# MiRaCLeXeoN/sduss

Measured on AMD Instinct MI355X. Metric: images/sec (node), SDXL 1024^2 50-step, fixed prompt, CFG, higher is better.
Workload: dtype bf16; 1 GPU; SDXL-base-1.0 UNet 1024x1024 50-step Euler, CFG 5.0, 4 requests/step (denoiser batch 8) per GPU, is_sliced=False, random-init weights of the real architecture (2.57 B params), one data-parallel replica per GPU, no collective; resolution=1024, steps_per_image=50

## Files before the change

include/mxdenoise.h:

```cpp
#ifndef MXDENOISE_H
#define MXDENOISE_H

#include <stddef.h>
#include <stdint.h>

#ifdef __cplusplus
extern "C" {
#endif

enum { MX_F32 = 0, MX_F16 = 1, MX_BF16 = 2 };

const char* mx_last_error(void);
int mx_version(void);
#define MX_PROF_KINDS 12
int mx_profile_enable(int on);
int mx_profile_collect(double* out);
int mx_profile_records(double* out, int max_records);

size_t mx_groupnorm_halo_workspace_bytes(int N, int C, int cpg);
int mx_groupnorm_halo(void* stream, const void* x, const void* gamma, const void* beta, void* y,
                      int N, int C, int H, int W, int cpg, double eps, int padding,
                      const int32_t* latent_offset, int n_latents, const int32_t* patch_map,
                      const int32_t* padding_idx, int dtype, void* workspace);
int mx_halo_only(void* stream, const void* x, void* y, int N, int C, int H, int W,
// ... 43 lines not shown
  int lda, ldc, ldr, ldrb;
  int rows_per_batch;
  int flags;
  int seg, period, ldvt;
  int B, Hin, Win, Cin;
  int Hout, Wout;
  int stride;
  int up;
  int corner_patch;
  int a_batch_rows, a_row_off, c_batch_rows, c_row_off;
  const float* gate;
  int ldg;
  float out_scale;
  const float* rms_wq;
  const float* rms_wk;
  float rms_eps;
  int vhalo;
  const void* a2;
  int lda2, k_split;
  const float* ln_stats;
  const float* ln_colsum;
  int ln_slabs;
  float ln_eps;
  float* stats_out;
  const mx_gemm_seg* segs;
  int n_segs;
  int splitk;
  const float* ln_final;
  float* ln_final_out;
  unsigned* ln_final_cnt;
  float* gn_part_out;
  int cin_valid;
} mx_gemm_desc;

int mx_gemm(void* stream, const mx_gemm_desc* d);
int mx_gemm_launches(const mx_gemm_desc* d);
int mx_gemm_stats_slabs(const mx_gemm_desc* d);
int mx_gemm_ln_prefers_pass(const mx_gemm_desc* d);
int mx_gemm_ln_final_supported(const mx_gemm_desc* d);
int mx_gemm_gn_partials_supported(const mx_gemm_desc* d, int conv);
enum { MX_LN_ROUTES_PATCH_PARALLEL = 1, MX_LN_ROUTES_PATCH_CACHE = 2, MX_LN_ROUTES_TICKETS = 4 };
int mx_unet_ln_routes(int M, int C, int layers, int n_groups, int flags, int routes[4]);
enum { MX_FORM_TILE_GENERIC = 0, MX_FORM_TILE_256 = 1, MX_FORM_TILE_128 = 2, MX_FORM_PERSISTENT_256 = 3, MX_FORM_SMALL_M = 4, MX_FORM_CONV_SMALL_N = 5, MX_FORM_CONV_SMALL_CIN = 6 };
int mx_gemm_form(const mx_gemm_desc* d, int conv);
int mx_gemm_kernel_name(const mx_gemm_desc* d, int conv, int launch, char* buf, int cap);
int mx_gemm_kernel_names(char* buf, int cap);
int mx_attention_kernel_name(int B, int H, int Lq, int Lk, int ldo, int prescaled, int causal, int bias, int key_chunk, int force_cross, char* buf, int cap);
int mx_attention_kernel_names(char* buf, int cap);
#define MX_STATS_PITCH(slabs) (((slabs) + 3) & ~3)
int mx_row_stats(void* stream, const void* x, int ldx, float* stats, int M, int C);
int mx_conv3x3(void* stream, const mx_gemm_desc* d);
int mx_conv3x3_halo_serves(const mx_gemm_desc* d);
int mx_conv3x3_halo(void* stream, const mx_gemm_desc* d);
int mx_gemm_splitk(const mx_gemm_desc* d, int conv);
void mx_gemm_release_scratch(void* stream, int all);

#define MX_VT_POS(key) (((key) & ~12) | (((key) & 4) << 1) | (((key) & 8) >> 1))
#define MX_VT_LD(Lk) (((Lk) + 15) / 16 * 16)

int mx_attention(void* stream, const void* q, int ldq, const void* k, int ldk, const void* vt, int ldvt,
                 int64_t vt_batch_stride, void* o, int ldo, int B, int H, int Lq, int Lk, float scale);
#define MX_ATTN_QSCALE(scale) ((scale) * 1.4426950408889634f)
int mx_attention_prescaled(void* stream, const void* q, int ldq, const void* k, int ldk, const void* vt, int ldvt,
                           int64_t vt_batch_stride, void* o, int ldo, int B, int H, int Lq, int Lk);
int mx_attention_cross_prescaled(void* stream, const void* q, int ldq, const void* k, int ldk, const void* vt, int ldvt,
                                 int64_t vt_batch_stride, void* o, int ldo, int B, int H, int Lq, int Lk);
typedef struct mx_attn_problem {
  const void* q; const void* k; const void* vt; void* o;
  int64_t vt_batch_stride;
  int B, Lq, Lk, ldvt;
} mx_attn_problem;
int mx_attention_prescaled_grouped(void* stream, const mx_attn_problem* probs, int n, int ldq, int ldk, int ldo, int H);
int mx_attention_prescaled_bias(void* stream, const void* q, int ldq, const void* k, int ldk, const void* vt, int ldvt,
                                int64_t vt_batch_stride, void* o, int ldo, int B, int H, int Lq, int Lk, const float* bias, int ldb);
int mx_attention_prescaled_causal(void* stream, const void* q, int ldq, const void* k, int ldk, const void* vt, int ldvt,
                                  int64_t vt_batch_stride, void* o, int ldo, int B, int H, int L);

int mx_layernorm(void* stream, const void* x, void* y, const float* gamma, const float* beta,
                 int M, int C, float eps);

int mx_rmsnorm(void* stream, const void* x, void* y, const float* w, int M, int C, float eps);

int mx_layernorm_mod(void* stream, const void* x, void* y, void* y2, const float* scale, const float* shift,
                     const float* scale2, const float* shift2, int ldmod, int M, int C, int rows_per_batch, float eps);
int mx_layernorm_mod_grouped(void* stream, const void* x, void* y, void* y2, const float* scale, const float* shift, const float* scale2,
                             const float* shift2, int ldmod, int C, float eps, const int* batches, const int* rows_per_batch, int n);
int mx_rmsnorm_heads(void* stream, void* x, int ld, int nbatch, int rows_per_batch, int batch_rows, int row_off,
                     int heads_total, int heads_q, const float* wq, const float* wk, float eps, float q_scale);

size_t mx_groupnorm_nhwc_workspace_bytes(int B, int H, int W, int C);
int mx_groupnorm_nhwc(void* stream, const void* x, void* y, const float* gamma, const float* beta,
                      int B, int H, int W, int C, int groups, float eps, int silu, int patch,
                      void* workspace);

int mx_groupnorm_nhwc_cat(void* stream, const void* x, int C1, const void* x2, void* y, const float* gamma, const float* beta,
                          int B, int H, int W, int C, int groups, float eps, int silu, int patch, void* workspace);
int mx_groupnorm_nhwc_from_partials(void* stream, const void* x, void* y, const float* gamma, const float* beta, int B, int H, int W, int C, int groups, float eps,
                                    int silu, const float* part, int chunk, const float* add_bias, const float* add_rowbias, int ldrb, void* workspace);

typedef struct mx_gn_problem { const void* x; const void* x2; void* y; int B, H, W; } mx_gn_problem;
size_t mx_groupnorm_nhwc_grouped_workspace_bytes(const mx_gn_problem* probs, int n, int C);
int mx_groupnorm_nhwc_grouped(void* stream, const mx_gn_problem* probs, int n, int C1, const float* gamma, const float* beta, int C, int groups,
                              float eps, int silu, int patch, void* workspace);

typedef struct mx_unet_config {
  int in_channels, out_channels;
// ... 358 lines not shown
```

sduss_amd/csrc/conv_halo.hip:

```cpp
#include "common.h"
#include "../../include/mxdenoise.h"
#include "gemm_args.h"
#include "gemm_dma_loader.h"

#include <type_traits>

namespace mx {

constexpr int HALO_BN = 160;
constexpr int HALO_WSTAGE_BYTES = HALO_BN * DMA_BK * 2;
constexpr int HALO_ZERO_BYTES = 256;
__host__ __device__ constexpr int halo_lines(int W) { return (256 / W + 2) * W; }
__host__ __device__ constexpr int halo_xbuf_bytes(int W) { return halo_lines(W) * DMA_BK * 2; }
__host__ __device__ constexpr int halo_lds_bytes(int W) { return 2 * halo_xbuf_bytes(W) + 3 * HALO_WSTAGE_BYTES + HALO_ZERO_BYTES; }

template <int W, bool VEC>
__global__ __launch_bounds__(512, 2) void conv_halo_kernel(const GemmArgs pk) {
  constexpr int BN = HALO_BN, MI = 4, NI = BN / 32;
  constexpr int LINES = halo_lines(W);
  constexpr int XBUF = halo_xbuf_bytes(W);
  constexpr int XN = LINES * 8 / 512;
  constexpr int WCH = BN * 8, WI = 3;
  constexpr int WRING = 2 * XBUF, ZERO = WRING + 3 * HALO_WSTAGE_BYTES;
  static_assert(W == 32 || W == 64, "a tile is whole image rows of 32 or 64 pixels");
  static_assert(LINES * 8 % 512 == 0 && XBUF % 256 == 0, "whole DMA instructions; buffers keep the bank half of a line");
  __shared__ __attribute__((aligned(256))) char smem[halo_lds_bytes(W)];

  const GemmArgs& p = pk;
  int tm, tn;
  gemm_tile_of_block(blockIdx.x, p.M / 256, p.N / BN, p.xcd_map, tm, tn);
  const int tid = threadIdx.x;
  const int lane = tid & 63;
  const int wave = __builtin_amdgcn_readfirstlane(tid >> 6);
  const int wm = wave >> 1;
  const int wn = wave & 1;
  const bool group_b = wave >= 4;
  const int cs = tid & 7;
  const int nchunks = p.Cin / DMA_BK;
  const char* zero = reinterpret_cast<const char*>(g_zero_page);

  const int m0 = tm * 256, n0 = tn * BN;
  const int hw = p.Hin * p.Win;
  const int img = m0 / hw;
  const int y0 = (m0 - img * hw) / W;
  const char* xsrc[XN];
#pragma unroll
  for (int i = 0; i < XN; ++i) {
    const int P = (i * 512 + tid) >> 3;
    const int sr = P / W, x = P - sr * W;
    const int iy = y0 - 1 + sr;
    const bool ok = iy >= 0 && iy < p.Hin;
    const long off = (((long)img * p.Hin + iy) * W + x) * (long)p.Cin * 2;
    xsrc[i] = (ok ? reinterpret_cast<const char*>(p.a) + off : zero) + swz(P, cs) * 16;
  }
  const char* wsrc[WI];
#pragma unroll
  for (int i = 0; i < WI; ++i) {
    int q = i * 512 + tid;
    if (q >= WCH) q -= WCH;
    const int row = q >> 3;
    wsrc[i] = reinterpret_cast<const char*>(p.w) + ((long)(n0 + row) * p.K + swz(row, cs) * 8) * 2;
  }
  const long w_tap_step = (long)p.Cin * 2, w_chunk_step = DMA_BK * 2 - 8 * (long)p.Cin * 2;

  auto issue_x = [&](int buf, int i) __attribute__((always_inline)) {
    glds16(xsrc[i], smem + buf * XBUF + (i * 512 + wave * 64) * 16);
  };
  auto advance_x = [&](int next_chunk) __attribute__((always_inline)) {
#pragma unroll
    for (int i = 0; i < XN; ++i) xsrc[i] = next_chunk < nchunks ? xsrc[i] + DMA_BK * 2 : zero + lane * 16;
  };
  auto issue_w = [&](int stage) __attribute__((always_inline)) {
#pragma unroll
    for (int i = 0; i < WI; ++i) {
      const int qb = (i * 512 + wave * 64 >= WCH) ? i * 512 + wave * 64 - WCH : i * 512 + wave * 64;
      glds16(wsrc[i], smem + WRING + stage * HALO_WSTAGE_BYTES + qb * 16);
    }
  };
  auto step_w = [&](long step) __attribute__((always_inline)) {
#pragma unroll
    for (int i = 0; i < WI; ++i) wsrc[i] += step;
  };
  auto to_next_chunk_w = [&](bool last) __attribute__((always_inline)) {
#pragma unroll
    for (int i = 0; i < WI; ++i) wsrc[i] = last ? zero + lane * 16 : wsrc[i] + w_chunk_step;
  };

  const int fr = lane & 15;
  const int fq = lane >> 4;
  unsigned wrd[2];
  unsigned xrd[3][2];
  unsigned zrd[3][2];
#pragma unroll
  for (int ks = 0; ks < 2; ++ks) {
    const int wrow = wn * (BN / 2) + fr;
    wrd[ks] = (unsigned)(WRING + wrow * 128 + swz(wrow, ks * 4 + fq) * 16);
#pragma unroll
    for (int d = 0; d < 3; ++d) {
      const int line = wm * 64 + fr + d - 1;
      const int key = ((fr + d - 1) >> 1) & 7;
      const int rel = line * 128 + ((ks * 4 + fq) ^ key) * 16;
      xrd[d][ks] = (unsigned)rel;
      zrd[d][ks] = (unsigned)(ZERO + (rel & 255));
    }
  }
  const bool lane_left = fr == 0, lane_right = fr == 15;

  if (tid < HALO_ZERO_BYTES / 16) *reinterpret_cast<u32x4*>(smem + ZERO + tid * 16) = u32x4{0u, 0u, 0u, 0u};

#pragma unroll
  for (int i = 0; i < XN; ++i) issue_x(0, i);
  advance_x(1);
  issue_w(0); step_w(w_tap_step);
  issue_w(1); step_w(w_tap_step);
  wait_vmcnt<WI>();

  f32x4 acc[NI][MI];
#pragma unroll
  for (int i = 0; i < NI; ++i)
#pragma unroll
    for (int j = 0; j < MI; ++j) acc[i][j] = f32x4{0.f, 0.f, 0.f, 0.f};
  float ln_rstd[MI];
#pragma unroll
  for (int j = 0; j < MI; ++j) ln_rstd[j] = 1.0f;
  asm volatile("s_waitcnt lgkmcnt(0)" ::: "memory");
  MX_BAR();
  if (group_b) MX_BAR();

  for (int cc = 0; cc < nchunks; ++cc) {
    const int cur = cc & 1, nxt = cur ^ 1;
    const unsigned xb = (unsigned)(cur * XBUF);
    const bool last = cc + 1 == nchunks;
    auto phase = [&](auto tc) __attribute__((always_inline)) {
      constexpr int T = decltype(tc)::value;
      constexpr int dy = T / 3 - 1, dx = T % 3 - 1, d = dx + 1;
      bf16x8 wf[2][NI], xf[2][MI];
#pragma unroll
      for (int ks = 0; ks < 2; ++ks) {
#pragma unroll
        for (int i = 0; i < NI; ++i) wf[ks][i] = *reinterpret_cast<const bf16x8*>(smem + wrd[ks] + (T % 3) * HALO_WSTAGE_BYTES + i * (16 * 128));
#pragma unroll
        for (int j = 0; j < MI; ++j) {
          unsigned a = xb + xrd[d][ks] + (unsigned)((dy + 1) * W * 128 + j * (16 * 128));
          if (dx == -1 && (j * 16) % W == 0) a = lane_left ? zrd[d][ks] : a;
          if (dx == 1 && (j * 16 + 16) % W == 0) a = lane_right ? zrd[d][ks] : a;
          xf[ks][j] = *reinterpret_cast<const bf16x8*>(smem + a);
        }
      }
      int nx = 0;
#pragma unroll
      for (int i = 0; i < XN; ++i)
        if ((i * 7) / (XN - 1) == T) { issue_x(nxt, i); ++nx; }
      issue_w((T + 2) % 3);
      if (T == 6) to_next_chunk_w(last);
      else step_w(T > 6 && last ? 0 : w_tap_step);
      if (T == 8) advance_x(cc + 2);
      if (nx == 0) wait_vmcnt<WI>(); else if (nx == 1) wait_vmcnt<WI + 1>(); else wait_vmcnt<WI + 2>();
      asm volatile("s_waitcnt lgkmcnt(0)" ::: "memory");
      __builtin_amdgcn_sched_barrier(0);
      MX_BAR();
      __builtin_amdgcn_s_setprio(1);
#pragma unroll
      for (int ks = 0; ks < 2; ++ks)
#pragma unroll
        for (int i = 0; i < NI; ++i)
#pragma unroll
          for (int j = 0; j < MI; ++j) acc[i][j] = __builtin_amdgcn_mfma_f32_16x16x32_bf16(wf[ks][i], xf[ks][j], acc[i][j], 0, 0, 0);
      __builtin_amdgcn_s_setprio(0);
      MX_BAR();
    };
    phase(std::integral_constant<int, 0>{}); phase(std::integral_constant<int, 1>{}); phase(std::integral_constant<int, 2>{});
    phase(std::integral_constant<int, 3>{}); phase(std::integral_constant<int, 4>{}); phase(std::integral_constant<int, 5>{});
    phase(std::integral_constant<int, 6>{}); phase(std::integral_constant<int, 7>{}); phase(std::integral_constant<int, 8>{});
  }
  if (!group_b) MX_BAR();

  gemm_epilogue_regs<NI, MI, false, VEC, true, true, 0, true, false>(p, acc, m0 + wm * 16 * MI, n0 + wn * (BN / 2), fr, fq, ln_rstd);
  if (p.gn_part != nullptr) gemm_gn_partials<NI, MI>(p, acc, m0 + wm * 16 * MI, n0 + wn * (BN / 2), fr, fq);
  wait_vmcnt<0>();
}

int conv_halo_lds_bytes(int width) { return width == 32 ? halo_lds_bytes(32) : width == 64 ? halo_lds_bytes(64) : 0; }

int launch_conv_halo(hipStream_t s, const GemmArgs& a, bool vec) {
  const dim3 grid((a.M / 256) * (a.N / HALO_BN)), block(512);
  if (a.Win == 32) {
    if (vec) hipLaunchKernelGGL((conv_halo_kernel<32, true>), grid, block, 0, s, a);
    else hipLaunchKernelGGL((conv_halo_kernel<32, false>), grid, block, 0, s, a);
    return 0;
  }
  if (a.Win == 64) {
    if (vec) hipLaunchKernelGGL((conv_halo_kernel<64, true>), grid, block, 0, s, a);
    else hipLaunchKernelGGL((conv_halo_kernel<64, false>), grid, block, 0, s, a);
    return 0;
  }
  return 1;
}

}
```

sduss_amd/csrc/gemm_dispatch.cpp:

```cpp
#include <algorithm>
#include <cstdlib>

#include <mutex>
#include <unordered_map>

#include "common.h"
#include "../../include/mxdenoise.h"
#include "gemm_args.h"
#include "gemm_forms.h"

namespace mx {

int launch_generic(hipStream_t s, const GemmArgs& a, int form);
int launch_v2(hipStream_t s, const GemmArgs& a, int form);
int launch_v5(hipStream_t s, const GemmArgs& a, int form);
int launch_v4(hipStream_t s, const GemmArgs& a, int form);
int launch_small_m(hipStream_t s, const GemmArgs& a, int form);
int launch_conv_small_n(hipStream_t s, const GemmArgs& a, int form);
int launch_conv_small_cin(hipStream_t s, const GemmArgs& a, int form);
bool small_m_serves(const mx_gemm_desc* d, bool conv);
int small_m_form(long N, long K, int flags);
bool conv_small_n_serves(const mx_gemm_desc* d);
bool conv_small_cin_serves(const mx_gemm_desc* d);

// ... 425 lines not shown
                                     : "gemm: no kernel instantiation serves this descriptor");
  GemmArgs a;
  fill_args(d, conv, r, a);
  hipStream_t s = (hipStream_t)stream;
  if (r.splitk > 1) {
    SplitKScratch sk;
    MX_CHECK(splitk_scratch(s, sk), "gemm: the split-K scratch (96 MB per stream) could not be allocated; set mx_gemm_desc.splitk = 1 to run unsplit");
    a.splitk = r.splitk; a.sk_ws = sk.ws; a.sk_cnt = sk.cnt;
  }
  if (prof_enabled()) {
    const double kk = conv ? 9.0 * d->Cin : (double)d->K;
    const double Mt = (double)rows_of(d);
    double in_elems = conv ? 0 : Mt * d->K;
    for (int i = 0; conv && i < problems_of(d); ++i) { const mx_gemm_seg g = problem_of(d, i); in_elems += (double)g.B * g.Hin * g.Win * d->Cin; }
    const double flops = 2.0 * Mt * (double)d->N * kk;
    const double bytes = 2.0 * (in_elems + (double)d->N * d->K + Mt * d->N);
    const int kind = r.bn == 256 ? PROF_GEMM_V4_256 : r.bn ? (conv ? PROF_CONV_V2_160 : PROF_GEMM_V2_160) + (r.bn == 160 ? 0 : 2) : (conv ? PROF_CONV128 : PROF_GEMM128) + (d->N % 128 == 0 ? 0 : 1);
    prof_begin(s, kind, flops, bytes, (int)Mt, d->N, (int)kk);
  }
  int bad = 1;
  switch (r.family) {
    case FAM_GENERIC: bad = launch_generic(s, a, r.form); break;
    case FAM_ROWS_128: bad = launch_v2(s, a, r.form); break;
    case FAM_ROWS_256: bad = launch_v5(s, a, r.form); break;
    case FAM_PERSISTENT_256: bad = launch_v4(s, a, r.form); break;
    case FAM_SMALL_M: bad = launch_small_m(s, a, r.form); break;
    case FAM_CONV_SMALL_N: bad = launch_conv_small_n(s, a, r.form); break;
    case FAM_CONV_SMALL_CIN: bad = launch_conv_small_cin(s, a, r.form); break;
  }
  MX_CHECK(bad == 0, "gemm: a family's launcher was handed a form outside its list");
  prof_end(s);
  MX_LAUNCH_CHECK();
  return 0;
}

static int run(void* stream, const mx_gemm_desc* d, bool conv) {
  MX_CHECK(d != nullptr, "gemm: null descriptor");
  MX_CHECK(d->n_segs >= 0 && d->n_segs <= MX_MAX_SEGS && (d->n_segs == 0 || d->segs != nullptr), "gemm: bad n_segs / segs");
  GemmPlan p;
  (void)plan_of(d, conv, p);
  for (int i = 0; i < p.n; ++i)
    if (int rc = launch(stream, p.d[i], conv, p.r[i])) return rc;
  return 0;
}

static bool plan_of_variant(const mx_gemm_desc* d, bool stats, GemmPlan& p) {
  if (!d) return false;
  mx_gemm_desc q = *d;
  if (!stats) q.ln_stats = nullptr;
  q.stats_out = !stats ? nullptr : d->stats_out ? d->stats_out : reinterpret_cast<float*>(16);
  return plan_of(&q, false, p);
}

int launch_conv_halo(hipStream_t s, const GemmArgs& a, bool vec);
int conv_halo_lds_bytes(int width);

static int conv_halo_serves(const mx_gemm_desc* d) {
  if (!d || d->n_segs != 0 || d->stride != 1 || d->up != 0 || d->vhalo != 0 || d->corner_patch != 0) return 0;
  if (d->Cin <= 0 || d->Cin % 64 != 0 || d->Cin > 8192 || d->K != 9 * d->Cin || d->cin_valid != 0) return 0;
  if (d->N <= 0 || d->N % 160 != 0) return 0;
  if (d->B <= 0 || d->Hin <= 0 || d->Hout != d->Hin || d->Wout != d->Win || (long)d->Hin * d->Win % 256 != 0) return 0;
  if ((long)d->B * d->Hin * d->Win != d->M) return 0;
  if (d->flags != 0 || d->gate || d->out_scale != 0.f || d->splitk > 1) return 0;
  if (d->rows_per_batch != 0 && d->rows_per_batch != d->Hin * d->Win) return 0;
  if (d->ldc % 8 != 0 || ((uintptr_t)d->c & 15) != 0) return 0;
  if (d->residual && (d->ldr % 8 != 0 || ((uintptr_t)d->residual & 15) != 0)) return 0;
  static const int kNotFaster[][3] = {{32, 640, 1280}, {64, 320, 640}};
  for (const auto& s : kNotFaster) if (d->Win == s[0] && d->Cin == s[1] && d->N == s[2]) return 0;
  return conv_halo_lds_bytes(d->Win);
}

static int run_conv_halo(void* stream, const mx_gemm_desc* d) {
  MX_CHECK(d != nullptr, "conv3x3_halo: null descriptor");
  MX_CHECK(conv_halo_serves(d) > 0, "conv3x3_halo: the descriptor is not served (mx_conv3x3_halo_serves); run mx_conv3x3");
  if (int rc = validate(d, true)) return rc;
  MX_CHECK(!d->stats_out && !d->ln_final_out, "conv3x3_halo: no row statistics");
  if (d->gn_part_out)
    MX_CHECK(!d->residual && (!d->rowbias || d->rows_per_batch % 64 == 0) && ((uintptr_t)d->gn_part_out & 15) == 0,
             "conv3x3_halo: gn_part_out needs an epilogue of bias (+ row bias) only and 16-byte alignment");
  GemmRoute r;
  r.bn = 160; r.rows = 256;
  GemmArgs a;
  fill_args(d, true, r, a);
  hipStream_t s = (hipStream_t)stream;
  if (prof_enabled()) {
    const double kk = 9.0 * d->Cin, Mt = (double)d->M;
    prof_begin(s, PROF_CONV_V2_160, 2.0 * Mt * (double)d->N * kk, 2.0 * (Mt * d->Cin + (double)d->N * d->K + Mt * d->N), d->M, d->N, (int)kk);
  }
  MX_CHECK(launch_conv_halo(s, a, d->rowbias != nullptr) == 0, "conv3x3_halo: no instantiation for this image width");
  prof_end(s);
  MX_LAUNCH_CHECK();
  return 0;
}

}

extern "C" int mx_conv3x3_halo_serves(const mx_gemm_desc* d) { return mx::conv_halo_serves(d); }
extern "C" int mx_conv3x3_halo(void* stream, const mx_gemm_desc* d) { return mx::run_conv_halo(stream, d); }
extern "C" int mx_gemm(void* stream, const mx_gemm_desc* d) { return mx::run(stream, d, false); }
extern "C" int mx_conv3x3(void* stream, const mx_gemm_desc* d) { return mx::run(stream, d, true); }
extern "C" void mx_gemm_release_scratch(void* stream, int all) { mx::splitk_release((hipStream_t)stream, all != 0); }

extern "C" int mx_gemm_launches(const mx_gemm_desc* d) { mx::GemmPlan p; return mx::plan_of(d, false, p) ? p.n : 1; }
extern "C" int mx_gemm_form(const mx_gemm_desc* d, int conv) { mx::GemmPlan p; return mx::plan_of(d, conv != 0, p) ? (int)p.r[0].family : MX_FORM_TILE_GENERIC; }
extern "C" int mx_gemm_splitk(const mx_gemm_desc* d, int conv) { mx::GemmPlan p; return mx::plan_of(d, conv != 0, p) ? p.r[0].splitk : 0; }
extern "C" int mx_gemm_gn_partials_supported(const mx_gemm_desc* d, int conv) { mx::GemmPlan p; return mx::plan_of(d, conv != 0, p) && p.r[0].gn_part; }
extern "C" int mx_gemm_stats_slabs(const mx_gemm_desc* d) { mx::GemmPlan p; return mx::plan_of_variant(d, true, p) ? p.r[0].stats_slabs : 0; }
extern "C" int mx_gemm_ln_final_supported(const mx_gemm_desc* d) { mx::GemmPlan p; return mx::plan_of_variant(d, true, p) && p.r[0].ln_final_out; }
extern "C" int mx_gemm_ln_prefers_pass(const mx_gemm_desc* d) { mx::GemmPlan p; return mx::plan_of_variant(d, false, p) && p.r[0].bn == 256; }
extern "C" int mx_gemm_kernel_name(const mx_gemm_desc* d, int conv, int launch, char* buf, int cap) {
  mx::GemmPlan p;
  if (launch < 0 || !mx::plan_of(d, conv != 0, p)) return -1;
  if (launch >= p.n) return 0;
  if (p.r[launch].form < 0) return -1;
  return mx::copy_name(mx::kGemmKernelNames[p.r[launch].form], buf, cap);
}
extern "C" int mx_gemm_kernel_names(char* buf, int cap) { return mx::join_names(mx::kGemmKernelNames, mx::GK_COUNT, buf, cap); }
```

sduss_amd/csrc/unet_sdxl.cpp:

```cpp
#include <hip/hip_runtime.h>

#include <algorithm>
#include <cstring>
#include <functional>
#include <map>
#include <string>
#include <vector>

#include "../../include/mxdenoise.h"
#include "common.h"
#include "graph_cache.h"
#include "ln_route.h"
#include "patch_cache.h"
#include "plan_base.h"

namespace mx {
int launch_prep_latent(hipStream_t s, const void* in, int dtype, void* out, int B, int Cin, int HW, int CP);
int launch_nhwc_to_nchw(hipStream_t s, const void* in, void* out, int dtype, int B, int C, int HW, int ld);
int launch_time_embed(hipStream_t s, const float* timesteps, const void* text_embeds, const float* time_ids,
                      void* tsin, void* addin, int B, int d0, int text_dim, int da);
int launch_concat(hipStream_t s, const void* a, const void* b, void* out, long M, int C1, int C2);
size_t gn_workspace_exact(int B, int H, int W, int C, int patch);
int launch_sq_diff_partial(hipStream_t s, const void* a, const void* b, long elems_per_sample, int B, double* partial, const int* slot = nullptr);
int launch_gn_pp_partial(hipStream_t s, const void* x, int C1, const void* x2, int B, int H, int W, int C, int groups, void* workspace, double* sums);
// ... 294 lines not shown
      case LnVia::Slabs:
        d.ln_stats = st.buf; d.ln_slabs = st.slabs;
        for (int g = 0; g < d.n_segs; ++g) segs[g].ln_stats = st.buf + row0[g] * MX_STATS_PITCH(st.slabs) * 2;
        break;
    }
    d.ln_colsum = colsum; d.ln_eps = u->cfg.layer_norm_eps;
  }
  bool linear(const Linear& l) {
    mx_gemm_desc d; std::memset(&d, 0, sizeof(d));
    d.out_scale = l.out_scale;
    if (l.a2) { d.a2 = l.a2; d.lda2 = l.lda2; d.k_split = l.lda; }
    d.a = l.a; d.lda = l.lda; d.w = wb(l.stem + ".weight", (size_t)l.N * l.K); d.bias = wf(l.stem + ".bias", l.N);
    d.c = l.c; d.ldc = l.ldc; d.M = l.M; d.N = l.N; d.K = l.K; d.residual = l.residual; d.ldr = l.ldr; d.flags = l.flags;
    if (l.ln_via != LnVia::Pass) use_ln(d, *l.ln, l.stem + ".colsum", l.ln_via);
    if (l.stats_via != LnVia::Pass) return gemm_with_stats(d, *l.stats_out, l.stats_via);
    return gemm(d, false);
  }
  int conv_cin_valid = 0;
  bool conv(const Conv& c) {
    const bf16_t* x = c.in.padded ? c.in.padded : c.in.t;
    const int Cin = c.Cin, Cout = c.Cout, stride = c.stride, up = c.up;
    mx_gemm_desc d; std::memset(&d, 0, sizeof(d));
    d.vhalo = c.in.padded ? 1 : 0;
    const int Hv = c.Hin << up, Wv = c.Win << up;
    d.a = x; d.w = wb(c.prefix + ".weight", (size_t)Cout * 9 * Cin); d.bias = wf(c.prefix + ".bias", Cout);
    d.c = c.out; d.ldc = Cout; d.B = gB[0]; d.Hin = c.Hin; d.Win = c.Win; d.Cin = Cin;
    d.Hout = (Hv + stride - 1) / stride; d.Wout = (Wv + stride - 1) / stride; d.stride = stride; d.up = up;
    d.corner_patch = c.corner_patch;
    d.M = gB[0] * d.Hout * d.Wout; d.N = Cout; d.K = 9 * Cin;
    d.rowbias = c.rowbias; d.ldrb = c.ldrb; d.rows_per_batch = d.Hout * d.Wout;
    d.residual = c.residual; d.ldr = Cout;
    mx_gemm_seg sg[MX_MAX_SEGS];
    if (ng > 1) {
      std::memset(sg, 0, sizeof(sg));
      long in0 = 0, out0 = 0;
      for (int g = 0; g < ng; ++g) {
        mx_gemm_seg& q = sg[g];
        q.B = gB[g]; q.Hin = ch[g]; q.Win = cw[g];
        q.Hout = ((ch[g] << up) + stride - 1) / stride; q.Wout = ((cw[g] << up) + stride - 1) / stride;
        q.M = gB[g] * q.Hout * q.Wout; q.rows_per_batch = q.Hout * q.Wout;
        q.a = x + in0 * Cin; q.c = c.out + out0 * Cout;
        q.residual = c.residual ? (const bf16_t*)c.residual + out0 * Cout : nullptr;
        q.rowbias = c.rowbias ? c.rowbias + (long)gb0[g] * c.ldrb : nullptr;
        in0 += (long)gB[g] * ch[g] * cw[g]; out0 += q.M;
      }
      d.segs = sg; d.n_segs = ng;
    }
    if (c.gn_part && c.gn_done && ng == 1 && mx_gemm_gn_partials_supported(&d, 1)) { d.gn_part_out = c.gn_part; *c.gn_done = true; }
    d.cin_valid = conv_cin_valid;
    if (mx_conv3x3_halo_serves(&d) && mx_gemm_form(&d, 1) == MX_FORM_TILE_256) {
      if (!ok()) return false;
      if (quiet()) return true;
      if (mx_conv3x3_halo(stream, &d)) return fail(std::string("conv3x3_halo: ") + mx_last_error());
      return true;
    }
    return gemm(d, true);
  }
  bool groupnorm(const bf16_t* x, bf16_t* y, const std::string& prefix, int h, int wd, int C, float eps, bool silu, int patch,
                 const bf16_t* x2 = nullptr, int C1 = 0) {
    if (!ok()) return false;
    const size_t m = ar.mark();
    mx_gn_problem pr[MX_MAX_SEGS];
    long r0 = 0;
    for (int k = 0; k < ng; ++k) {
      pr[k].x = x + r0 * (x2 ? C1 : C); pr[k].x2 = x2 ? x2 + r0 * (C - C1) : nullptr; pr[k].y = y + r0 * C;
      pr[k].B = gB[k]; pr[k].H = ch[k]; pr[k].W = cw[k];
      r0 += (long)gB[k] * ch[k] * cw[k];
    }
    const size_t need = ng > 1 ? mx_groupnorm_nhwc_grouped_workspace_bytes(pr, ng, C) : mx::gn_workspace_exact(gB[0], h, wd, C, patch);
    void* ws = ar.alloc(need);
    if (!ws) return fail("workspace too small");
    const float* g = wf(prefix + ".weight", C); const float* b = wf(prefix + ".bias", C);
    if (ok() && !quiet()) {
      if (mx_groupnorm_nhwc_grouped(stream, pr, ng, x2 ? C1 : C, g, b, C, u->cfg.norm_num_groups, eps, silu ? 1 : 0, patch, ws))
        fail(std::string("groupnorm: ") + mx_last_error());
    }
    ar.release(m);
    return ok();
  }
  bool groupnorm_from_partials(const bf16_t* x, bf16_t* y, const std::string& prefix, int h, int wd, int C, float eps, bool silu, const float* part,
                               const float* add_bias, const float* add_rowbias, int ldrb) {
    if (!ok()) return false;
    const size_t m = ar.mark();
    void* ws = ar.alloc(mx::gn_workspace_exact(gB[0], h, wd, C, 0));
    if (!ws) return fail("workspace too small");
    const float* g = wf(prefix + ".weight", C); const float* b = wf(prefix + ".bias", C);
    if (ok() && !quiet()) {
      if (mx_groupnorm_nhwc_from_partials(stream, x, y, g, b, gB[0], h, wd, C, u->cfg.norm_num_groups, eps, silu ? 1 : 0, part, 64, add_bias, add_rowbias, ldrb, ws))
        fail(std::string("groupnorm: ") + mx_last_error());
    }
    ar.release(m);
    return ok();
  }
  bool attention(const bf16_t* q, int ldq, const bf16_t* k, int ldk, const bf16_t* vt, int ldvt, long vt_bstride, bf16_t* o,
                 int ldo, int heads, int Lq, int Lk) {
    if (!ok()) return false;
    if (quiet()) return true;
    if (mx_attention_prescaled(stream, q, ldq, k, ldk, vt, ldvt, vt_bstride, o, ldo, B, heads, Lq, Lk))
      return fail(std::string("attention: ") + mx_last_error());
    return true;
  }
  bool attention_grouped(const mx_attn_problem* pr, int ldq, int ldk, int ldo, int heads) {
    if (!ok()) return false;
    if (quiet()) return true;
    if (mx_attention_prescaled_grouped(stream, pr, ng, ldq, ldk, ldo, heads)) return fail(std::string("attention: ") + mx_last_error());
    return true;
// ... 1010 lines not shown
```

sduss_amd/lib.py:

```python
from __future__ import annotations

import ctypes as C
import os
from typing import Optional

_HERE = os.path.dirname(os.path.abspath(__file__))
LIB_PATH = os.path.join(_HERE, "libmxdenoise.so")

MX_F32, MX_F16, MX_BF16 = 0, 1, 2
EPI_SILU, EPI_GEGLU, EPI_OUT_F32, EPI_QKV, EPI_GELU_TANH, EPI_RES_BCAST, EPI_RMSNORM, EPI_GELU, EPI_QUICK_GELU, EPI_GEGLU_TANH = 1, 2, 4, 8, 16, 32, 64, 128, 256, 512


class MxError(RuntimeError):
    """Raised for every non-zero status of the C ABI (the reference's launcher only printed
    cudaGetLastError and went on -- norm_silu_concat.cu:434-437; SURVEY.md section 8b asks to raise)."""


MAX_SEGS = 4


class GemmSeg(C.Structure):
    _fields_ = [
        ("a", C.c_void_p), ("a2", C.c_void_p), ("c", C.c_void_p), ("residual", C.c_void_p), ("vt", C.c_void_p), ("rowbias", C.c_void_p),
        ("gate", C.c_void_p), ("ln_stats", C.c_void_p), ("stats_out", C.c_void_p),
# ... 142 lines not shown
                ("keep", C.c_void_p), ("sigma", C.c_void_p), ("latents", C.c_void_p), ("io_dtype", C.c_int),
                ("scaling_factor", C.c_float), ("shift_factor", C.c_float)]


class InpaintRows(C.Structure):
    _fields_ = [("k", C.c_int), ("slot", C.c_void_p), ("init", C.c_void_p), ("noise", C.c_void_p), ("mask", C.c_void_p)]


MX_SAMPLER_EULER, MX_SAMPLER_DPMPP_2M, MX_SAMPLER_AB2 = 0, 1, 2
SAMPLERS = {"euler": MX_SAMPLER_EULER, "dpmpp_2m": MX_SAMPLER_DPMPP_2M, "ab2": MX_SAMPLER_AB2}


MX_SAMPLER_EULER_A, MX_SAMPLER_DPMPP_2M_SDE = 3, 4
STOCHASTIC_SAMPLERS = {"euler_a": MX_SAMPLER_EULER_A, "dpmpp_2m_sde": MX_SAMPLER_DPMPP_2M_SDE}
MX_NOISE_INIT, MX_NOISE_START, MX_NOISE_STEP, MX_NOISE_POSTERIOR = 0, 1, 2, 3


class NoiseRows(C.Structure):
    _fields_ = [("cn", C.c_void_p), ("seed", C.c_void_p), ("step", C.c_void_p)]


class MultistepRows(C.Structure):
    _fields_ = [("kind", C.c_void_p), ("coef", C.c_void_p), ("hist", C.c_void_p)]


LORA_NO_VECTOR = (1 << 64) - 1
LORA_MAX_RANK = 512


class LoraTerm(C.Structure):
    _fields_ = [("w_off", C.c_uint64), ("N", C.c_int), ("K", C.c_int), ("row0", C.c_int), ("rows", C.c_int), ("up", C.c_void_p),
                ("down_t", C.c_void_p), ("R", C.c_int), ("scale", C.c_float), ("colsum_off", C.c_uint64), ("bias_off", C.c_uint64),
                ("dbias", C.c_void_p)]


class WeightEntry(C.Structure):
    _fields_ = [("name", C.c_char_p), ("offset", C.c_uint64), ("bytes", C.c_uint64)]


_vp, _i, _f, _d, _i64, _sz = C.c_void_p, C.c_int, C.c_float, C.c_double, C.c_int64, C.c_size_t
SYMBOLS = {
    "mx_last_error": (C.c_char_p, []),
    "mx_version": (_i, []),
    "mx_profile_enable": (_i, [_i]),
    "mx_profile_collect": (_i, [C.POINTER(C.c_double)]),
    "mx_profile_records": (_i, [C.POINTER(C.c_double), _i]),
    "mx_groupnorm_halo_workspace_bytes": (_sz, [_i, _i, _i]),
    "mx_groupnorm_halo": (_i, [_vp, _vp, _vp, _vp, _vp, _i, _i, _i, _i, _i, _d, _i, _vp, _i, _vp, _vp, _i, _vp]),
    "mx_halo_only": (_i, [_vp, _vp, _vp, _i, _i, _i, _i, _vp, _i]),
    "mx_gemm": (_i, [_vp, C.POINTER(GemmDesc)]),
    "mx_conv3x3": (_i, [_vp, C.POINTER(GemmDesc)]),
    "mx_conv3x3_halo": (_i, [_vp, C.POINTER(GemmDesc)]),
    "mx_conv3x3_halo_serves": (_i, [C.POINTER(GemmDesc)]),
    "mx_gemm_stats_slabs": (_i, [C.POINTER(GemmDesc)]),
    "mx_gemm_ln_prefers_pass": (_i, [C.POINTER(GemmDesc)]),
    "mx_row_stats": (_i, [_vp, _vp, _i, _vp, _i, _i]),
    "mx_attention": (_i, [_vp, _vp, _i, _vp, _i, _vp, _i, _i64, _vp, _i, _i, _i, _i, _i, _f]),
    "mx_attention_prescaled": (_i, [_vp, _vp, _i, _vp, _i, _vp, _i, _i64, _vp, _i, _i, _i, _i, _i]),
    "mx_attention_cross_prescaled": (_i, [_vp, _vp, _i, _vp, _i, _vp, _i, _i64, _vp, _i, _i, _i, _i, _i]),
    "mx_layernorm": (_i, [_vp, _vp, _vp, _vp, _vp, _i, _i, _f]),
    "mx_groupnorm_nhwc_workspace_bytes": (_sz, [_i, _i, _i, _i]),
    "mx_groupnorm_nhwc": (_i, [_vp, _vp, _vp, _vp, _vp, _i, _i, _i, _i, _i, _f, _i, _i, _vp]),
    "mx_groupnorm_nhwc_cat": (_i, [_vp, _vp, _i, _vp, _vp, _vp, _vp, _i, _i, _i, _i, _i, _f, _i, _i, _vp]),
    "mx_attention_prescaled_grouped": (_i, [_vp, C.POINTER(AttnProblem), _i, _i, _i, _i, _i]),
    "mx_groupnorm_nhwc_grouped_workspace_bytes": (_sz, [C.POINTER(GnProblem), _i, _i]),
    "mx_groupnorm_nhwc_grouped": (_i, [_vp, C.POINTER(GnProblem), _i, _i, _vp, _vp, _i, _i, _f, _i, _i, _vp]),
    "mx_unet_workspace_bytes_mixed": (_sz, [_vp, C.POINTER(UNetGroup), _i, _i]),
    "mx_unet_forward_mixed": (_i, [_vp, _vp, C.POINTER(UNetGroup), _i, _i, _vp, _vp, _vp, _vp, _i, _i, _vp, _sz]),
    "mx_unet_forward_mixed_trace": (_i, [_vp, _vp, C.POINTER(UNetGroup), _i, _i, _vp, _vp, _vp, _vp, _i, _i, _vp, _sz, C.c_char_p, _vp, _sz]),
    "mx_mmdit_workspace_bytes_mixed": (_sz, [_vp, C.POINTER(UNetGroup), _i, _i]),
    "mx_mmdit_forward_mixed": (_i, [_vp, _vp, C.POINTER(UNetGroup), _i, _i, _vp, _vp, _vp, _i, _vp, _sz]),
    "mx_unet_create": (_vp, [C.POINTER(UNetConfigC)]),
    "mx_unet_destroy": (None, [_vp]),
    "mx_unet_set_context_key": (_i, [_vp, C.c_uint64]),
    "mx_unet_context_stats": (_i, [_vp, C.POINTER(C.c_long), C.POINTER(C.c_long)]),
    "mx_unet_set_weights": (_i, [_vp, _vp, C.c_uint64, C.POINTER(WeightEntry), _i]),
    "mx_unet_workspace_bytes": (_sz, [_vp, _i, _i, _i, _i]),
    "mx_unet_validate": (_i, [_vp, _i, _i, _i, _i]),
    "mx_unet_forward": (_i, [_vp, _vp, _vp, _i, _vp, _vp, _vp, _vp, _vp, _i, _i, _i, _i, _i, _vp, _sz]),
    "mx_forest_predict": (_i, [_vp, _vp, _vp, _vp, _vp, _vp, _i, _vp, _i, _i, _vp]),
    "mx_skip_counters_bytes": (_sz, [_i, _i, _i]),
    "mx_skip_decide_host": (_i, [C.POINTER(DeviceForestC), _i, _i, _i, _i, _vp, _vp, _vp, _vp, _vp, _vp, _vp, _vp, _vp]),
    "mx_skip_decide_device": (_i, [_vp, C.POINTER(SkipDecideArgs)]),
    "mx_pc_image_copy": (_i, [_vp, _vp, _vp, _vp, _i, _i, _i, _i64, _i, _vp, _i, _vp, _i64, _i]),
    "mx_pc_rows_load_stats": (_i, [_vp, _vp, _vp, _vp, _i, _i, _i, _i64, _vp, _vp, _vp, _f, _i64]),
    "mx_pc_gather": (_i, [_vp, _vp, _i, _i, _vp, _vp, _i, _vp, _i, _i, _i, _i, _i]),
    "mx_pc_scatter": (_i, [_vp, _vp, _i, _i, _i, _vp, _i64, _vp, _i, _vp, _i, _i]),
    "mx_pc_patch_store": (_i, [_vp, _vp, _vp, _i64, _i, _vp, _i, _vp, _i, _i]),
    "mx_pc_patch_sq_diff": (_i, [_vp, _vp, _vp, _i64, _i, _vp, _i, _vp, _i, _i, _vp]),
    "mx_pc_range_copy": (_i, [_vp, _vp, _vp, _i64, _i, _vp, _i, _i, _i64]),
    "mx_pc_range_sq_diff": (_i, [_vp, _vp, _vp, _i64, _i, _vp, _i, _vp]),
    "mx_sq_diff_partial": (_i, [_vp, _vp, _vp, _i64, _i, _vp, _vp]),
    "mx_copy_rows": (_i, [_vp, _vp, _vp, _sz, _i, _vp, _i]),
    "mx_mmdit_workspace_bytes_pp": (_sz, [_vp, _i, _i, _i, _i, _i]),
    "mx_mmdit_pp_state_bytes": (_sz, [_vp, _i, _i, _i, _i, _i]),
    "mx_mmdit_forward_pp": (_i, [_vp, _vp, _vp, _i, _vp, _vp, _vp, _vp, _i, _i, _i, _i, _vp, _vp, _vp, _sz]),
    "mx_mmdit_pp_comm_plan": (_i, [_vp, _i, _i, _i, _i, _vp]),
    "mx_unet_pp_state_bytes": (_sz, [_vp, _i, _i, _i, _i, _i]),
    "mx_unet_forward_pp_stale": (_i, [_vp, _vp, _vp, _i, _vp, _vp, _vp, _vp, _vp, _i, _i, _i, _i, _vp, _vp, _vp, _sz]),
    "mx_unet_block_cache_bytes": (_sz, [_vp, _i, _i, _i]),
    "mx_gemm_splitk": (_i, [_vp, _i]),
    "mx_gemm_release_scratch": (None, [_vp, _i]),
    "mx_gemm_ln_final_supported": (_i, [C.POINTER(GemmDesc)]),
    "mx_gemm_launches": (_i, [C.POINTER(GemmDesc)]),
    "mx_gemm_gn_partials_supported": (_i, [C.POINTER(GemmDesc), _i]),
    "mx_unet_ln_routes": (_i, [_i, _i, _i, _i, _i, C.POINTER(_i)]),
# ... 164 lines not shown
```

Baseline: 1.434 images/s.

## Extend halo-staged 3x3 conv kernel to 128-wide images via half-row tiles

Adds a half-row variant of the LDS halo conv kernel for 128-pixel-wide feature maps. Each 256-row tile covers four half-rows of 64 pixels plus a one-pixel side column, loaded by a single wave into a small extra LDS buffer so the horizontal taps read real neighbours instead of zeros. The UNet dispatch now sends the 128x128 SDXL convs through this path instead of the generic implicit-GEMM conv. The aim is to cut redundant global loads of the im2col input at the highest resolution, at the cost of extra LDS, an extra DMA and wait on one wave, and a non-contiguous output mapping in the epilogue.

New measurement: 1.451 images/s, median of 6. 1.2% higher.

```diff
diff --git a/include/mxdenoise.h b/include/mxdenoise.h
--- a/include/mxdenoise.h
+++ b/include/mxdenoise.h
@@ -119,6 +119,8 @@
 int mx_conv3x3(void* stream, const mx_gemm_desc* d);
 int mx_conv3x3_halo_serves(const mx_gemm_desc* d);
 int mx_conv3x3_halo(void* stream, const mx_gemm_desc* d);
+int mx_conv3x3_halfrow_serves(const mx_gemm_desc* d);
+int mx_conv3x3_halfrow(void* stream, const mx_gemm_desc* d);
 int mx_gemm_splitk(const mx_gemm_desc* d, int conv);
 void mx_gemm_release_scratch(void* stream, int all);
 
diff --git a/sduss_amd/csrc/conv_halo.hip b/sduss_amd/csrc/conv_halo.hip
--- a/sduss_amd/csrc/conv_halo.hip
+++ b/sduss_amd/csrc/conv_halo.hip
@@ -12,19 +12,32 @@
 constexpr int HALO_ZERO_BYTES = 256;
 __host__ __device__ constexpr int halo_lines(int W) { return (256 / W + 2) * W; }
 __host__ __device__ constexpr int halo_xbuf_bytes(int W) { return halo_lines(W) * DMA_BK * 2; }
-__host__ __device__ constexpr int halo_lds_bytes(int W) { return 2 * halo_xbuf_bytes(W) + 3 * HALO_WSTAGE_BYTES + HALO_ZERO_BYTES; }
-
-template <int W, bool VEC>
+constexpr int HALO_SIDE_BYTES = 1024;
+__host__ __device__ constexpr int halo_lds_bytes(int W, bool half) {
+  return 2 * halo_xbuf_bytes(W) + 3 * HALO_WSTAGE_BYTES + HALO_ZERO_BYTES + (half ? 2 * HALO_SIDE_BYTES : 0);
+}
+__host__ __device__ constexpr int halo_pieces_in_tap(int XN, int T) {
+  int n = 0;
+  for (int i = 0; i < XN; ++i) n += (i * 7) / (XN - 1) == T ? 1 : 0;
+  return n;
+}
+
+template <int W, bool HALF, bool VEC>
 __global__ __launch_bounds__(512, 2) void conv_halo_kernel(const GemmArgs pk) {
   constexpr int BN = HALO_BN, MI = 4, NI = BN / 32;
+  constexpr int IW = HALF ? 2 * W : W;
   constexpr int LINES = halo_lines(W);
   constexpr int XBUF = halo_xbuf_bytes(W);
   constexpr int XN = LINES * 8 / 512;
   constexpr int WCH = BN * 8, WI = 3;
-  constexpr int WRING = 2 * XBUF, ZERO = WRING + 3 * HALO_WSTAGE_BYTES;
+  constexpr int WRING = 2 * XBUF, ZERO = WRING + 3 * HALO_WSTAGE_BYTES, SIDE = ZERO + HALO_ZERO_BYTES;
+  constexpr int SIDE_TAP = 3, SIDE_WAVE = 0;
   static_assert(W == 32 || W == 64, "a tile is whole image rows of 32 or 64 pixels");
+  static_assert(!HALF || W == 64, "half rows: a 128-wide image");
+  static_assert(!HALF || (256 / W + 2) * 8 <= 64, "the side column is one wave-wide DMA");
+  static_assert(halo_lds_bytes(W, HALF) <= 160 * 1024, "LDS of one workgroup");
   static_assert(LINES * 8 % 512 == 0 && XBUF % 256 == 0, "whole DMA instructions; buffers keep the bank half of a line");
-  __shared__ __attribute__((aligned(256))) char smem[halo_lds_bytes(W)];
+  __shared__ __attribute__((aligned(256))) char smem[halo_lds_bytes(W, HALF)];
 
   const GemmArgs& p = pk;
   int tm, tn;
@@ -41,8 +54,11 @@
 
   const int m0 = tm * 256, n0 = tn * BN;
   const int hw = p.Hin * p.Win;
-  const int img = m0 / hw;
-  const int y0 = (m0 - img * hw) / W;
+  const int half = HALF ? tm & 1 : 0;
+  const int mrows0 = HALF ? (tm >> 1) * 512 : m0;
+  const int img = mrows0 / hw;
+  const int y0 = (mrows0 - img * hw) / IW;
+  const int xo = half * W;
   const char* xsrc[XN];
 #pragma unroll
   for (int i = 0; i < XN; ++i) {
@@ -50,8 +66,17 @@
     const int sr = P / W, x = P - sr * W;
     const int iy = y0 - 1 + sr;
     const bool ok = iy >= 0 && iy < p.Hin;
-    const long off = (((long)img * p.Hin + iy) * W + x) * (long)p.Cin * 2;
+    const long off = (((long)img * p.Hin + iy) * IW + xo + x) * (long)p.Cin * 2;
     xsrc[i] = (ok ? reinterpret_cast<const char*>(p.a) + off : zero) + swz(P, cs) * 16;
+  }
+  const char* xside = zero;
+  if constexpr (HALF) {
+    const int sl = lane >> 3;
+    const int iy = y0 - 1 + sl;
+    const bool ok = sl < 256 / W + 2 && iy >= 0 && iy < p.Hin;
+    const int xs = half ? xo - 1 : xo + W;
+    const long off = (((long)img * p.Hin + iy) * IW + xs) * (long)p.Cin * 2;
+    xside = (ok ? reinterpret_cast<const char*>(p.a) + off : zero) + (cs ^ (half ? 7 : 0)) * 16;
   }
   const char* wsrc[WI];
 #pragma unroll
@@ -69,6 +94,10 @@
   auto advance_x = [&](int next_chunk) __attribute__((always_inline)) {
 #pragma unroll
     for (int i = 0; i < XN; ++i) xsrc[i] = next_chunk < nchunks ? xsrc[i] + DMA_BK * 2 : zero + lane * 16;
+    if constexpr (HALF) xside = next_chunk < nchunks ? xside + DMA_BK * 2 : zero + lane * 16;
+  };
+  auto issue_side = [&](int buf) __attribute__((always_inline)) {
+    glds16(xside, smem + SIDE + buf * HALO_SIDE_BYTES);
   };
   auto issue_w = [&](int stage) __attribute__((always_inline)) {
 #pragma unroll
@@ -102,6 +131,7 @@
       const int rel = line * 128 + ((ks * 4 + fq) ^ key) * 16;
       xrd[d][ks] = (unsigned)rel;
       zrd[d][ks] = (unsigned)(ZERO + (rel & 255));
+      if constexpr (HALF) { if (d == (half ? 0 : 2)) zrd[d][ks] = (unsigned)(SIDE + wm * 128 + (rel & 127)); }
     }
   }
   const bool lane_left = fr == 0, lane_right = fr == 15;
@@ -110,6 +140,7 @@
 
 #pragma unroll
   for (int i = 0; i < XN; ++i) issue_x(0, i);
+  if constexpr (HALF) { if (wave == SIDE_WAVE) issue_side(0); }
   advance_x(1);
   issue_w(0); step_w(w_tap_step);
   issue_w(1); step_w(w_tap_step);
@@ -134,6 +165,8 @@
     auto phase = [&](auto tc) __attribute__((always_inline)) {
       constexpr int T = decltype(tc)::value;
       constexpr int dy = T / 3 - 1, dx = T % 3 - 1, d = dx + 1;
+      constexpr int NX = halo_pieces_in_tap(XN, T);
+      const unsigned side_off = HALF && dx != 0 && (dx < 0) == (half != 0) ? (unsigned)(cur * HALO_SIDE_BYTES + (dy + 1) * 128) : 0u;
       bf16x8 wf[2][NI], xf[2][MI];
 #pragma unroll
       for (int ks = 0; ks < 2; ++ks) {
@@ -142,20 +175,21 @@
 #pragma unroll
         for (int j = 0; j < MI; ++j) {
           unsigned a = xb + xrd[d][ks] + (unsigned)((dy + 1) * W * 128 + j * (16 * 128));
-          if (dx == -1 && (j * 16) % W == 0) a = lane_left ? zrd[d][ks] : a;
-          if (dx == 1 && (j * 16 + 16) % W == 0) a = lane_right ? zrd[d][ks] : a;
+          if (dx == -1 && (j * 16) % W == 0) a = lane_left ? zrd[d][ks] + side_off : a;
+          if (dx == 1 && (j * 16 + 16) % W == 0) a = lane_right ? zrd[d][ks] + side_off : a;
           xf[ks][j] = *reinterpret_cast<const bf16x8*>(smem + a);
         }
       }
-      int nx = 0;
 #pragma unroll
       for (int i = 0; i < XN; ++i)
-        if ((i * 7) / (XN - 1) == T) { issue_x(nxt, i); ++nx; }
+        if ((i * 7) / (XN - 1) == T) issue_x(nxt, i);
+      constexpr bool side_tap = HALF && T == SIDE_TAP;
+      if constexpr (side_tap) { if (wave == SIDE_WAVE) issue_side(nxt); }
       issue_w((T + 2) % 3);
       if (T == 6) to_next_chunk_w(last);
       else step_w(T > 6 && last ? 0 : w_tap_step);
       if (T == 8) advance_x(cc + 2);
-      if (nx == 0) wait_vmcnt<WI>(); else if (nx == 1) wait_vmcnt<WI + 1>(); else wait_vmcnt<WI + 2>();
+      if (side_tap && wave == SIDE_WAVE) wait_vmcnt<WI + NX + 1>(); else wait_vmcnt<WI + NX>();
       asm volatile("s_waitcnt lgkmcnt(0)" ::: "memory");
       __builtin_amdgcn_sched_barrier(0);
       MX_BAR();
@@ -175,23 +209,33 @@
   }
   if (!group_b) MX_BAR();
 
-  gemm_epilogue_regs<NI, MI, false, VEC, true, true, 0, true, false>(p, acc, m0 + wm * 16 * MI, n0 + wn * (BN / 2), fr, fq, ln_rstd);
-  if (p.gn_part != nullptr) gemm_gn_partials<NI, MI>(p, acc, m0 + wm * 16 * MI, n0 + wn * (BN / 2), fr, fq);
+  const int m_wave0 = HALF ? img * hw + (y0 + wm) * IW + xo : m0 + wm * 16 * MI;
+  gemm_epilogue_regs<NI, MI, false, VEC, true, true, 0, true, false>(p, acc, m_wave0, n0 + wn * (BN / 2), fr, fq, ln_rstd);
+  if (p.gn_part != nullptr) gemm_gn_partials<NI, MI>(p, acc, m_wave0, n0 + wn * (BN / 2), fr, fq);
   wait_vmcnt<0>();
 }
 
-int conv_halo_lds_bytes(int width) { return width == 32 ? halo_lds_bytes(32) : width == 64 ? halo_lds_bytes(64) : 0; }
-
-int launch_conv_halo(hipStream_t s, const GemmArgs& a, bool vec) {
+int conv_halo_lds_bytes(int width, bool half_rows) {
+  if (half_rows) return width == 128 ? halo_lds_bytes(64, true) : 0;
+  return width == 32 ? halo_lds_bytes(32, false) : width == 64 ? halo_lds_bytes(64, false) : 0;
+}
+
+int launch_conv_halo(hipStream_t s, const GemmArgs& a, bool vec, bool half_rows) {
   const dim3 grid((a.M / 256) * (a.N / HALO_BN)), block(512);
+  if (half_rows) {
+    if (a.Win != 128) return 1;
+    if (vec) hipLaunchKernelGGL((conv_halo_kernel<64, true, true>), grid, block, 0, s, a);
+    else hipLaunchKernelGGL((conv_halo_kernel<64, true, false>), grid, block, 0, s, a);
+    return 0;
+  }
   if (a.Win == 32) {
-    if (vec) hipLaunchKernelGGL((conv_halo_kernel<32, true>), grid, block, 0, s, a);
-    else hipLaunchKernelGGL((conv_halo_kernel<32, false>), grid, block, 0, s, a);
+    if (vec) hipLaunchKernelGGL((conv_halo_kernel<32, false, true>), grid, block, 0, s, a);
+    else hipLaunchKernelGGL((conv_halo_kernel<32, false, false>), grid, block, 0, s, a);
     return 0;
   }
   if (a.Win == 64) {
-    if (vec) hipLaunchKernelGGL((conv_halo_kernel<64, true>), grid, block, 0, s, a);
-    else hipLaunchKernelGGL((conv_halo_kernel<64, false>), grid, block, 0, s, a);
+    if (vec) hipLaunchKernelGGL((conv_halo_kernel<64, false, true>), grid, block, 0, s, a);
+    else hipLaunchKernelGGL((conv_halo_kernel<64, false, false>), grid, block, 0, s, a);
     return 0;
   }
   return 1;
diff --git a/sduss_amd/csrc/gemm_dispatch.cpp b/sduss_amd/csrc/gemm_dispatch.cpp
--- a/sduss_amd/csrc/gemm_dispatch.cpp
+++ b/sduss_amd/csrc/gemm_dispatch.cpp
@@ -501,27 +501,38 @@
   return plan_of(&q, false, p);
 }
 
-int launch_conv_halo(hipStream_t s, const GemmArgs& a, bool vec);
-int conv_halo_lds_bytes(int width);
+int launch_conv_halo(hipStream_t s, const GemmArgs& a, bool vec, bool half_rows);
+int conv_halo_lds_bytes(int width, bool half_rows);
+
+static bool conv_staged_common(const mx_gemm_desc* d) {
+  if (!d || d->n_segs != 0 || d->stride != 1 || d->up != 0 || d->vhalo != 0 || d->corner_patch != 0) return false;
+  if (d->Cin <= 0 || d->Cin % 64 != 0 || d->Cin > 8192 || d->K != 9 * d->Cin || d->cin_valid != 0) return false;
+  if (d->N <= 0 || d->N % 160 != 0) return false;
+  if (d->B <= 0 || d->Hin <= 0 || d->Win <= 0 || d->Hout != d->Hin || d->Wout != d->Win) return false;
+  if ((long)d->B * d->Hin * d->Win != d->M) return false;
+  if (d->flags != 0 || d->gate || d->out_scale != 0.f || d->splitk > 1) return false;
+  if (d->rows_per_batch != 0 && d->rows_per_batch != d->Hin * d->Win) return false;
+  if (d->ldc % 8 != 0 || ((uintptr_t)d->c & 15) != 0) return false;
+  if (d->residual && (d->ldr % 8 != 0 || ((uintptr_t)d->residual & 15) != 0)) return false;
+  return true;
+}
 
 static int conv_halo_serves(const mx_gemm_desc* d) {
-  if (!d || d->n_segs != 0 || d->stride != 1 || d->up != 0 || d->vhalo != 0 || d->corner_patch != 0) return 0;
-  if (d->Cin <= 0 || d->Cin % 64 != 0 || d->Cin > 8192 || d->K != 9 * d->Cin || d->cin_valid != 0) return 0;
-  if (d->N <= 0 || d->N % 160 != 0) return 0;
-  if (d->B <= 0 || d->Hin <= 0 || d->Hout != d->Hin || d->Wout != d->Win || (long)d->Hin * d->Win % 256 != 0) return 0;
-  if ((long)d->B * d->Hin * d->Win != d->M) return 0;
-  if (d->flags != 0 || d->gate || d->out_scale != 0.f || d->splitk > 1) return 0;
-  if (d->rows_per_batch != 0 && d->rows_per_batch != d->Hin * d->Win) return 0;
-  if (d->ldc % 8 != 0 || ((uintptr_t)d->c & 15) != 0) return 0;
-  if (d->residual && (d->ldr % 8 != 0 || ((uintptr_t)d->residual & 15) != 0)) return 0;
+  if (!conv_staged_common(d) || (long)d->Hin * d->Win % 256 != 0) return 0;
   static const int kNotFaster[][3] = {{32, 640, 1280}, {64, 320, 640}};
   for (const auto& s : kNotFaster) if (d->Win == s[0] && d->Cin == s[1] && d->N == s[2]) return 0;
-  return conv_halo_lds_bytes(d->Win);
-}
-
-static int run_conv_halo(void* stream, const mx_gemm_desc* d) {
+  return conv_halo_lds_bytes(d->Win, false);
+}
+
+static int conv_halfrow_serves(const mx_gemm_desc* d) {
+  if (!conv_staged_common(d) || d->Win != 128 || d->Hin % 4 != 0) return 0;
+  return conv_halo_lds_bytes(d->Win, true);
+}
+
+static int run_conv_halo(void* stream, const mx_gemm_desc* d, bool half_rows) {
   MX_CHECK(d != nullptr, "conv3x3_halo: null descriptor");
-  MX_CHECK(conv_halo_serves(d) > 0, "conv3x3_halo: the descriptor is not served (mx_conv3x3_halo_serves); run mx_conv3x3");
+  if (half_rows) MX_CHECK(conv_halfrow_serves(d) > 0, "conv3x3_halfrow: the descriptor is not served (mx_conv3x3_halfrow_serves); run mx_conv3x3");
+  else MX_CHECK(conv_halo_serves(d) > 0, "conv3x3_halo: the descriptor is not served (mx_conv3x3_halo_serves); run mx_conv3x3");
   if (int rc = validate(d, true)) return rc;
   MX_CHECK(!d->stats_out && !d->ln_final_out, "conv3x3_halo: no row statistics");
   if (d->gn_part_out)
@@ -536,7 +547,7 @@
     const double kk = 9.0 * d->Cin, Mt = (double)d->M;
     prof_begin(s, PROF_CONV_V2_160, 2.0 * Mt * (double)d->N * kk, 2.0 * (Mt * d->Cin + (double)d->N * d->K + Mt * d->N), d->M, d->N, (int)kk);
   }
-  MX_CHECK(launch_conv_halo(s, a, d->rowbias != nullptr) == 0, "conv3x3_halo: no instantiation for this image width");
+  MX_CHECK(launch_conv_halo(s, a, d->rowbias != nullptr, half_rows) == 0, "conv3x3_halo: no instantiation for this image width");
   prof_end(s);
   MX_LAUNCH_CHECK();
   return 0;
@@ -545,7 +556,9 @@
 }
 
 extern "C" int mx_conv3x3_halo_serves(const mx_gemm_desc* d) { return mx::conv_halo_serves(d); }
-extern "C" int mx_conv3x3_halo(void* stream, const mx_gemm_desc* d) { return mx::run_conv_halo(stream, d); }
+extern "C" int mx_conv3x3_halo(void* stream, const mx_gemm_desc* d) { return mx::run_conv_halo(stream, d, false); }
+extern "C" int mx_conv3x3_halfrow_serves(const mx_gemm_desc* d) { return mx::conv_halfrow_serves(d); }
+extern "C" int mx_conv3x3_halfrow(void* stream, const mx_gemm_desc* d) { return mx::run_conv_halo(stream, d, true); }
 extern "C" int mx_gemm(void* stream, const mx_gemm_desc* d) { return mx::run(stream, d, false); }
 extern "C" int mx_conv3x3(void* stream, const mx_gemm_desc* d) { return mx::run(stream, d, true); }
 extern "C" void mx_gemm_release_scratch(void* stream, int all) { mx::splitk_release((hipStream_t)stream, all != 0); }
diff --git a/sduss_amd/csrc/unet_sdxl.cpp b/sduss_amd/csrc/unet_sdxl.cpp
--- a/sduss_amd/csrc/unet_sdxl.cpp
+++ b/sduss_amd/csrc/unet_sdxl.cpp
@@ -370,6 +370,12 @@
       if (!ok()) return false;
       if (quiet()) return true;
       if (mx_conv3x3_halo(stream, &d)) return fail(std::string("conv3x3_halo: ") + mx_last_error());
+      return true;
+    }
+    if (mx_conv3x3_halfrow_serves(&d) && mx_gemm_form(&d, 1) == MX_FORM_TILE_256) {
+      if (!ok()) return false;
+      if (quiet()) return true;
+      if (mx_conv3x3_halfrow(stream, &d)) return fail(std::string("conv3x3_halfrow: ") + mx_last_error());
       return true;
     }
     return gemm(d, true);
diff --git a/sduss_amd/lib.py b/sduss_amd/lib.py
--- a/sduss_amd/lib.py
+++ b/sduss_amd/lib.py
@@ -218,6 +218,8 @@
     "mx_conv3x3": (_i, [_vp, C.POINTER(GemmDesc)]),
     "mx_conv3x3_halo": (_i, [_vp, C.POINTER(GemmDesc)]),
     "mx_conv3x3_halo_serves": (_i, [C.POINTER(GemmDesc)]),
+    "mx_conv3x3_halfrow": (_i, [_vp, C.POINTER(GemmDesc)]),
+    "mx_conv3x3_halfrow_serves": (_i, [C.POINTER(GemmDesc)]),
     "mx_gemm_stats_slabs": (_i, [C.POINTER(GemmDesc)]),
     "mx_gemm_ln_prefers_pass": (_i, [C.POINTER(GemmDesc)]),
     "mx_row_stats": (_i, [_vp, _vp, _i, _vp, _i, _i]),
```
